# relf/egobox

Hardware: AMD Instinct MI355X
Metric: gp_fixed_theta_fits_per_sec (higher is better)
Workload: dtype f64; 1 GPU; dense GP fixed-theta fit (corr build + Cholesky + likelihood), sq-exp, n=16384 d=32, LHS + Griewank; theta sweep, 192 per step; n=16384, d=32, corr=SquaredExponential, mean=Constant, parallelism=sweep-dp1, fits_in_flight_per_gpu=16, lockstep_width=8

## Files before the change

### egobox_amd/csrc/egx_internal.h

```cpp
#pragma once
#include <hip/hip_runtime.h>
#include <stdint.h>
#include <string>

#include "../../include/egx_gp.h"
#include "schedule.h"

namespace egx {

void set_error(const std::string &msg);
#define EGX_HIP_CHECK(expr)                                                              \
    do {                                                                                 \
        hipError_t _e = (expr);                                                          \
        if (_e != hipSuccess) {                                                          \
            ::egx::set_error(std::string(#expr) + ": " + hipGetErrorString(_e));         \
            (void)hipGetLastError();  \
            return EGX_ERR_HIP;                                                          \
        }                                                                                \
    } while (0)

hipError_t dev_malloc_bytes(void **p, size_t bytes);
template <typename T>
inline hipError_t dev_malloc(T **p, size_t bytes) {
    return dev_malloc_bytes(reinterpret_cast<void **>(p), bytes);
// ... 125 lines not shown
    int rsplit = 1;
    int init = 0;
    const int *active = nullptr;
    double *means = nullptr;
    double *prec = nullptr;
    double *cst = nullptr;
    double *weights = nullptr;
    double *covs = nullptr;
    double *part = nullptr;
    double *lpn_part = nullptr;
    double *lbst = nullptr;
};
inline size_t gmm_part_len(int DP) { return (size_t)(DP / 4) * (DP / 4 + 1) / 2 * kGmmBlockAcc; }
size_t gmm_estep_lds_bytes(int DP, int k);
int launch_gmm_estep(hipStream_t s, const GmmLaunch &g);
int launch_gmm_mstep(hipStream_t s, const GmmLaunch &g, double reg_covar);

inline size_t dinv_doubles(int n_pad) { return (size_t)(n_pad / 64) * 4096 + (size_t)(n_pad / 64); }
struct GemmTrace {
    static constexpr int kMax = 192;
    hipEvent_t e0[kMax], e1[kMax];
    double flops[kMax];
    int used = 0;
    bool ready = false;
};
struct PotrfLookahead {
    hipStream_t s2 = nullptr, s3 = nullptr;
    hipEvent_t ev_lu = nullptr, ev_lur = nullptr, ev_panel = nullptr, ev_a = nullptr, ev_b = nullptr;
};
struct PotrfInverse {
    double *W = nullptr;
    int64_t ldw = 0, sW = 0;
    hipStream_t sw = nullptr;
    hipEvent_t ev_grp = nullptr, ev_done = nullptr;
};
struct GemmBatch {
    int count = 1;
    int64_t sC = 0, sA = 0, sB = 0;
    int sInfo = 0;
};
struct PotrfBatch {
    int count = 1;
    int64_t sM = 0, sD = 0;
    int sI = 0;
    int left = 0;
    int w_left = 0;
    int *sync = nullptr;
    int64_t sS = 0;
    int pipe = 0;
    int whole = 0;
    int flow = 0;
    int flow_tail = 0;
    int group_panels = 0;
    int seqs = 1;
};
int potrf_left_for(int n_pad, int lockstep);
int w_left_for(int n_pad, int lockstep);
PotrfSchedule schedule_for(int n_pad, int lockstep, int n_workspaces);
int potrf_group_panels(int n_pad);
struct TrsmBatch {
    int count = 1;
    int64_t sM = 0, sD = 0, sR = 0;
};
int launch_potrf(hipStream_t s, double *M, int64_t ld, int n_pad, int m_tot, double *dinv, int *info,
                 const PotrfLookahead *lk = nullptr, GemmTrace *trace = nullptr, const PotrfBatch *batch = nullptr,
                 const PotrfInverse *inv = nullptr);
int launch_trsm_rows(hipStream_t s, const double *M, int64_t ldm, int n_pad, const double *dinv,
                     double *RT, int64_t ldr, int m, int tri_rows = 0, const TrsmBatch *batch = nullptr);
int launch_identity_rows(hipStream_t s, double *W, int64_t ld, int n_pad, int count = 1, int64_t stride = 0);
int launch_syrk_uptri_neg(hipStream_t s, double *C, int64_t ldc, const double *W, int64_t ldw, int n,
                          const GemmBatch *batch = nullptr);
int launch_diag_tile_inverses(hipStream_t s, const double *M, int64_t ld, int n_pad, double *dinv);
struct SolveBatchPtrs {
    const double *M[kLockstepMax], *dinv[kLockstepMax];
    double *dW[kLockstepMax], *rhs[kLockstepMax], *vec[kLockstepMax];
};
inline size_t trsv_tail_doubles(int n_pad) { return 4 + (size_t)n_pad; }
inline size_t block_inverse_doubles(int n_pad) { return (size_t)((n_pad + kNB - 1) / kNB) * 65536 + trsv_tail_doubles(n_pad); }
long long pipe_timeout_ticks();
int launch_block_inverse(hipStream_t s, const SolveBatchPtrs &b, int count, int64_t ld, int n_pad);
int launch_trsv_t(hipStream_t s, const SolveBatchPtrs &b, int count, int64_t ld, int n_pad, bool per_block = false);
inline int launch_block_inverse(hipStream_t s, const double *M, int64_t ld, int n_pad, const double *dinv, double *Wall) {
    const SolveBatchPtrs b{{M}, {dinv}, {Wall}, {}, {}};
    return launch_block_inverse(s, b, 1, ld, n_pad);
}
inline int launch_trsv_t(hipStream_t s, const double *M, int64_t ld, int n_pad, double *Wall, double *v, double *xout,
                         bool per_block = false) {
    const SolveBatchPtrs b{{M}, {}, {Wall}, {v}, {xout}};
    return launch_trsv_t(s, b, 1, ld, n_pad, per_block);
}
int launch_gemm_nt_sub(hipStream_t s, double *C, int64_t ldc, const double *A, int64_t lda,
                       const double *B, int64_t ldb, int M, int N, int K, int lower, int ktri = 0,
                       bool *used_big_tile = nullptr, const int *info = nullptr, const GemmBatch *batch = nullptr,
                       int tag = 0);
size_t gram_scratch_doubles(int rows, int K);
int launch_gram_lower(hipStream_t s, const double *W, int64_t ldw, int rows, int K, double *Gneg, int64_t ldg, double *P);
int mfma_probe(double *max_abs_err);

size_t pipe_sync_ints(int n_pad, int m_tot);
int launch_potrf_pipe(hipStream_t s, double *M, int64_t ld, int n_pad, int m_tot, double *dinv, int *info,
                      const PotrfBatch &pb, int g0, int gw, int ext_need = 0, int shared_chip = 0);
int pipe_signal(hipStream_t s, const PotrfBatch &pb, int value);
int launch_potrf_flow(hipStream_t s, double *M, int64_t ld, int n_pad, int m_tot, double *dinv, int *info, const PotrfBatch &pb,
                      int col_base = 0);
bool flow_fits(int n_pad);
int pipe_enabled();
// ... 15 lines not shown
```

### egobox_amd/csrc/gp_host.hip

```cpp
#include "gp_handle.h"
#include "resource_pool.h"

namespace egx {

static thread_local std::string g_last_error;
static std::atomic<int> g_pipe_retry{[] { const char *e = std::getenv("EGX_PIPE_RETRY"); return e ? std::atoi(e) : 1; }()};
static std::atomic<int64_t> g_chain_aborts{0}, g_chain_retries{0};
void set_error(const std::string &msg) { g_last_error = msg; }
const std::string &last_error_string() { return g_last_error; }

}

using namespace egx;

namespace egx {

int set_device(const egx_gp *gp) {
    EGX_HIP_CHECK(hipSetDevice(gp->device));
    return EGX_SUCCESS;
}

struct StreamSet {
    hipStream_t stream = nullptr, inv_stream = nullptr, s2 = nullptr, s3 = nullptr;
};
// ... 278 lines not shown
    }
    egx_gp *gp = owners[0];
    Workspace &lead = *wss[0];
    hipStream_t st = lead.stream;
    PotrfInverse inv;
    if (W0) {
        inv.W = W0;
        inv.ldw = gp->n_pad;
        inv.sW = (int64_t)gp->n_pad * gp->n_pad;
        inv.sw = lead.inv_stream;
        inv.ev_grp = lead.ev_inv_grp;
        inv.ev_done = lead.ev_inv_done;
        EGX_RC(launch_identity_rows(inv.sw, W0, gp->n_pad, gp->n_pad, count, inv.sW));
    }
    for (int j = 0; j < count; j++) {
        Workspace &w = *wss[j];
        w.eval_stream = st;
        std::memcpy(w.h_coef, coefs[j].data(), sizeof(double) * coefs[j].size());
        EGX_HIP_CHECK(hipMemcpyAsync(w.d_coef, w.h_coef, sizeof(double) * coefs[j].size(), hipMemcpyHostToDevice, st));
    }
    EGX_HIP_CHECK(hipMemsetAsync(lead.d_info, 0, sizeof(int) * (size_t)count, st));
    EGX_HIP_CHECK(hipEventRecord(lead.ev[0], st));
    EvalBatchPtrs bp;
    for (int j = 0; j < count; j++) {
        Workspace &w = *wss[j];
        bp.xT[j] = owners[j]->d_xT, bp.coef[j] = w.d_coef, bp.rhsT[j] = owners[j]->d_rhsT, bp.xs[j] = w.d_xs, bp.M[j] = w.M;
        bp.h_diag[j] = w.h_diag, bp.h_rows[j] = w.h_rows, bp.h_info[j] = w.h_info, bp.d_info[j] = w.d_info;
    }
    const int front = launch_eval_front_batch(st, gp->corr, bp, count, gp->n_pad, gp->n, gp->d, hcols, gp->nugget, gp->ld, gp->n_pad,
                                              gp->rhs_pad, gp->q);
    if (front != EGX_SUCCESS && front != EGX_ERR_UNSUPPORTED) return front;
    if (front == EGX_ERR_UNSUPPORTED)
        for (int j = 0; j < count; j++) {
            Workspace &w = *wss[j];
            egx_gp *o = owners[j];
            EGX_RC(launch_corr_sym(st, gp->corr, o->d_xT, gp->n_pad, gp->n, gp->d, w.d_coef, hcols, gp->nugget, w.M, gp->ld,
                                   gp->n_pad, w.d_xs));
            EGX_RC(launch_fill_rows(st, w.M, gp->ld, gp->n_pad, gp->rhs_pad, o->d_rhsT, gp->n_pad, gp->q, gp->n_pad));
        }
    EGX_HIP_CHECK(hipEventRecord(lead.ev[1], st));
    int *lead_sync = dev_sync(gp, (int)(&lead - gp->ws.data()));
    PotrfBatch pb;
    pb.count = count;
    pb.sM = gp->stride_M;
    pb.sD = gp->stride_D;
    pb.sI = 1;
    pb.left = gp->sched.left;
    pb.w_left = gp->sched.w_left;
    pb.pipe = separate ? 0 : gp->sched.pipe;
    pb.whole = separate ? 0 : gp->sched.whole;
    pb.flow = separate || count > 1 || gp->group ? 0 : gp->sched.flow;
    pb.flow_tail = separate || count > 1 || gp->group ? 0 : gp->sched.flow_tail;
    pb.group_panels = gp->sched.group_panels;
    pb.seqs = gp->lockstep > 0 ? ((int)gp->ws.size() + gp->lockstep - 1) / gp->lockstep : 1;
    pb.sync = pb.pipe || pb.flow || pb.flow_tail ? lead_sync : nullptr;
    pb.sS = gp->stride_S;
    for (int j = 0; j < count; j++) {
        wss[j]->retry_hcols = hcols;
        wss[j]->retry_W = W0 ? W0 + (size_t)j * (size_t)gp->n_pad * gp->n_pad : nullptr;
        wss[j]->retry_ncoef = (int)coefs[j].size();
        wss[j]->retried = separate;
    }
    EGX_RC(launch_potrf(st, lead.M, gp->ld, gp->n_pad, gp->m_tot, lead.dinv, lead.d_info, lead.lk.s2 ? &lead.lk : nullptr,
                        &lead.trace, &pb, W0 ? &inv : nullptr));
    EGX_HIP_CHECK(hipEventRecord(lead.ev[2], st));
    EGX_RC(launch_eval_tail(st, bp, count, gp->ld, gp->n, gp->n_pad, gp->q, gp->gls_device ? 0 : 1, pb.sync));
    for (int j = 0; j < count; j++) {
        Workspace &w = *wss[j];
        w.gls_enqueued = gp->gls_device;
        if (gp->gls_device) {
            const int g = gp->rhs_pad;
            EGX_RC(launch_gram_lower(st, w.M + (size_t)gp->n_pad * gp->ld, gp->ld, g, gp->n_pad, w.d_gneg, g, w.d_gramP));
            EGX_RC(launch_gram_finish(st, w.d_gneg, w.d_gram, g, g, gp->q));
            EGX_HIP_CHECK(hipMemsetAsync(w.d_ginfo, 0, sizeof(int), st));
            EGX_RC(launch_potrf(st, w.d_gram, g, g, g, w.d_gdinv, w.d_ginfo));
            EGX_HIP_CHECK(hipMemcpyAsync(w.h_gram, w.d_gram, sizeof(double) * (size_t)g * g, hipMemcpyDeviceToHost, st));
            EGX_HIP_CHECK(hipMemcpyAsync(w.h_ginfo, w.d_ginfo, sizeof(int), hipMemcpyDeviceToHost, st));
        }
        w.sync_lead = pb.sync;
    }
    EGX_HIP_CHECK(hipEventRecord(lead.ev[3], st));
    return EGX_SUCCESS;
}

int enqueue_eval_group(egx_gp *gp, int w0, int count, const std::vector<double> *coefs, int hcols, double *W0) {
    std::vector<egx_gp *> owners((size_t)count, gp);
    std::vector<Workspace *> wss((size_t)count);
    for (int j = 0; j < count; j++) wss[(size_t)j] = &gp->ws[(size_t)(w0 + j)];
    return enqueue_eval_core(owners.data(), wss.data(), count, coefs, hcols, W0);
}
int enqueue_eval_members(egx_gp *const *gps, int count, const std::vector<double> *coefs, int hcols) {
    std::vector<Workspace *> wss((size_t)count);
    for (int j = 0; j < count; j++) wss[(size_t)j] = &gps[j]->ws[0];
    return enqueue_eval_core(gps, wss.data(), count, coefs, hcols, nullptr);
}

int enqueue_eval(egx_gp *gp, Workspace &w, const std::vector<double> &coef, int hcols) {
    return enqueue_eval_group(gp, (int)(&w - gp->ws.data()), 1, &coef, hcols);
}

static int finish_eval_device_gls(egx_gp *gp, Workspace &w, EvalResult &out, int keep) {
    const int n = gp->n, p = gp->p, n_pad = gp->n_pad, g = gp->rhs_pad;
    if (*w.h_ginfo != 0) return 1;
    const double *L = w.h_gram;
    double dmin = std::numeric_limits<double>::infinity(), dmax = 0.0;
    for (int i = 0; i < p; i++) {
// ... 1335 lines not shown
```

### egobox_amd/csrc/kernels_chol.hip

```cpp
#include "egx_internal.h"
#include "dev_mem.h"
#include "potf2_blocks.h"
#include "mfma_gemm_core.h"

#include <atomic>
#include <cstdlib>
#include <mutex>
#include <string>
#include <utility>
#include <vector>

namespace egx {


__device__ __forceinline__ double readlane_d(double v, int lane) {
    union {
        double d;
        int i[2];
    } u;
    u.d = v;
    u.i[0] = __builtin_amdgcn_readlane(u.i[0], lane);
    u.i[1] = __builtin_amdgcn_readlane(u.i[1], lane);
    return u.d;
}
// ... 323 lines not shown
            mma_quarter(a1, b1, 1);
            stage = st1;
        }
#ifdef EGX_STREAM_TRACE
        if (trp) trp[6] = wall_clock64(), trp[7] = clock64();
#endif
#pragma unroll
        for (int r = 0; r < 4; r++) asm volatile("" : "+v"(coff[r]));
#pragma unroll
        for (int mi = 0; mi < 4; mi++)
#pragma unroll
            for (int ni = 0; ni < 4; ni++)
#pragma unroll
                for (int r = 0; r < 4; r++) Ct[(int64_t)mi * 16 * ldc + ni * 16 + coff[r]] = -acc[mi][ni][r];
#ifdef EGX_STREAM_TRACE
        if (trp) {
            asm volatile("s_waitcnt vmcnt(0)" ::: "memory");
            trp[8] = wall_clock64();
        }
#endif
    }
}

#ifdef EGX_STREAM_TRACE
}
extern "C" long long egx_dev_stream_trace(int mode, long long *out, long long cap) {
    static auto &owned = *new egx::DevMem<long long>;
    static long long dcap = 0;
    long long *null = nullptr, *dbuf = owned.p;
    if (mode == 1) {
        owned.reset();
        dcap = cap;
        if (owned.alloc((size_t)(16 + egx::kStraceWords * cap)) != EGX_SUCCESS) return -1;
        dbuf = owned.p;
        (void)hipMemset(dbuf, 0, sizeof(long long) * (16 + egx::kStraceWords * cap));
        (void)hipMemcpy(dbuf + 1, &cap, sizeof(long long), hipMemcpyHostToDevice);
        if (hipMemcpyToSymbol(HIP_SYMBOL(egx::g_strace), &dbuf, sizeof(dbuf)) != hipSuccess) return -2;
        return 0;
    }
    (void)hipDeviceSynchronize();
    (void)hipMemcpyToSymbol(HIP_SYMBOL(egx::g_strace), &null, sizeof(null));
    if (!dbuf) return 0;
    long long taken = 0;
    (void)hipMemcpy(&taken, dbuf, sizeof(long long), hipMemcpyDeviceToHost);
    if (taken > dcap) taken = dcap;
    if (taken > cap) taken = cap;
    if (out && taken > 0) (void)hipMemcpy(out, dbuf + 16, sizeof(long long) * egx::kStraceWords * taken, hipMemcpyDeviceToHost);
    owned.reset();
    return taken;
}
namespace egx {
#endif

constexpr int TS = 64;
constexpr int TLD = 65;

template <int NW>
__device__ __forceinline__ void wg_inv_64(const double *T, const double *rd, double *X, int tid) {
    const int wave = tid >> 6, lane = tid & 63;
    const int frow = lane & 15, fk = lane >> 4;
#pragma unroll 1
    for (int cbk = 3; cbk >= 0; cbk--) {
        for (int rt = wave; rt < 4; rt += NW) {
            double *xt = X + (rt * 16 + fk) * TLD + cbk * 16 + frow;
            double4_t acc = double4_t{0.0, 0.0, 0.0, 0.0};
            if (rt == cbk) {
#pragma unroll
                for (int r = 0; r < 4; r++) acc[r] = (fk + 4 * r == frow) ? 1.0 : 0.0;
            } else if (rt > cbk) {
                for (int kb = cbk + 1; kb <= rt; kb++) {
                    const double *arow = X + (rt * 16 + frow) * TLD + kb * 16 + fk;
                    const double *bcol = T + (kb * 16 + fk) * TLD + cbk * 16 + frow;
#pragma unroll
                    for (int kk = 0; kk < 4; kk++)
                        acc = __builtin_amdgcn_mfma_f64_16x16x4f64(-arow[kk * 4], bcol[(kk * 4) * TLD], acc, 0, 0, 0);
                }
            }
#pragma unroll
            for (int r = 0; r < 4; r++) xt[(4 * r) * TLD] = acc[r];
        }
        __syncthreads();
        if (wave == 0) {
            double x[16];
#pragma unroll
            for (int c = 0; c < 16; c++) x[c] = X[lane * TLD + cbk * 16 + c];
#pragma unroll
            for (int c = 15; c >= 0; c--) {
                double sacc = x[c];
#pragma unroll
                for (int k = c + 1; k < 16; k++)
                    sacc = __builtin_fma(-x[k], T[(cbk * 16 + k) * TLD + cbk * 16 + c], sacc);
                x[c] = sacc * rd[cbk * 16 + c];
            }
#pragma unroll
            for (int c = 0; c < 16; c++) X[lane * TLD + cbk * 16 + c] = x[c];
        }
        __syncthreads();
    }
}


template <int NW>
__global__ __launch_bounds__(64 * NW, 1) void k_potf2_reg(double *__restrict__ D, int64_t ld, int nbk, double *__restrict__ lin,
                                                          int *__restrict__ info, int col0, int n_valid, int64_t bsD,
                                                          int64_t bsL, int bsI) {
    extern __shared__ __attribute__((aligned(16))) double sm[];
// ... 359 lines not shown
                                                        int K, double *__restrict__ P) {
    using S = GemmShape<64, 64, 32, 32, 256>;
    extern __shared__ __attribute__((aligned(16))) double smem[];
    const int t = blockIdx.x;
    int bx = (int)((sqrt(8.0 * t + 1.0) - 1.0) * 0.5);
    while (bx * (bx + 1) / 2 > t) bx--;
    while ((bx + 1) * (bx + 2) / 2 <= t) bx++;
    const int by = t - bx * (bx + 1) / 2;
    const int k0 = blockIdx.y * kc;
    int klen = K - k0;
    if (klen > kc) klen = kc;
    const int tid = threadIdx.x;
    double4_t acc[S::MT][S::NT];
#pragma unroll
    for (int mi = 0; mi < S::MT; mi++)
#pragma unroll
        for (int ni = 0; ni < S::NT; ni++) acc[mi][ni] = double4_t{0.0, 0.0, 0.0, 0.0};
    if (klen > 0)
        gemm_core<64, 64, 32, 32, 256>(W + (int64_t)bx * 64 * ldw + k0, ldw, W + (int64_t)by * 64 * ldw + k0, ldw, klen,
                                       acc, smem, tid);
    const int wave = tid >> 6, lane = tid & 63;
    const int r0 = bx * 64 + (wave / S::WAVES_N) * 32 + (lane >> 4);
    const int c0 = by * 64 + (wave % S::WAVES_N) * 32 + (lane & 15);
    double *out = P + (int64_t)blockIdx.y * rows * rows;
#pragma unroll
    for (int mi = 0; mi < S::MT; mi++)
#pragma unroll
        for (int ni = 0; ni < S::NT; ni++)
#pragma unroll
            for (int r = 0; r < 4; r++) out[(int64_t)(r0 + mi * 16 + 4 * r) * rows + (c0 + ni * 16)] = acc[mi][ni][r];
}

__global__ void k_gram_reduce(const double *__restrict__ P, int rows, int nsplit, double *__restrict__ Gneg, int64_t ldg) {
    const int j = blockIdx.x * blockDim.x + threadIdx.x, i = blockIdx.y;
    if (j >= rows || (j >> 6) > (i >> 6)) return;
    double sacc = 0.0;
    for (int sp = 0; sp < nsplit; sp++) sacc += P[((int64_t)sp * rows + i) * rows + j];
    Gneg[(int64_t)i * ldg + j] = -sacc;
}

static std::atomic<int> g_potrf_group{0};
static std::atomic<int> g_stream_min_tiles{128};
static std::atomic<int> g_gemm_small_max{1024};
static std::atomic<int> g_look_min_cols{3072};
static std::atomic<int> g_lur_side{1};
#ifdef EGX_TEST_HOOKS
static std::atomic<int> g_trsv_stall{0};
#define EGX_TRSV_STALL g_trsv_stall.load()
#else
#define EGX_TRSV_STALL 0
#endif
static std::atomic<int> g_trsv_fused{1};
static std::atomic<int> g_potrf_left{1};
constexpr int kTrsmGroupPanels = 4;
constexpr int kLurSideMinCols = 6144;

int chol_init() {
    static std::once_flag once;
    static int rc_once = EGX_SUCCESS;
    std::call_once(once, [] {
        if (const char *e = std::getenv("EGX_POTRF_GROUP")) {
            const int g = std::atoi(e);
            if (g >= 1 && g <= 8) g_potrf_group = g;
        }
        if (const char *e = std::getenv("EGX_GEMM_SMALL")) g_gemm_small_max = std::atoi(e);
        if (const char *e = std::getenv("EGX_STREAM_MIN")) g_stream_min_tiles = std::atoi(e) > 0 ? std::atoi(e) : 1;
        if (const char *e = std::getenv("EGX_LOOK_MIN")) g_look_min_cols = std::atoi(e);
        if (const char *e = std::getenv("EGX_LUR_SIDE")) g_lur_side = std::atoi(e);
        if (const char *e = std::getenv("EGX_TRSV_FUSED")) g_trsv_fused = std::atoi(e);
        if (const char *e = std::getenv("EGX_POTRF_LEFT")) g_potrf_left = std::atoi(e);
        auto set = [](const void *fn, int bytes) {
            hipError_t e = hipFuncSetAttribute(fn, hipFuncAttributeMaxDynamicSharedMemorySize, bytes);
            if (e != hipSuccess && rc_once == EGX_SUCCESS) {
                set_error(std::string("hipFuncSetAttribute: ") + hipGetErrorString(e));
                rc_once = EGX_ERR_HIP;
            }
        };
        set(reinterpret_cast<const void *>(&k_gemm_nt_sub<true, 128, 128, 32, 64, 512, true>), TrailShape::LDS_BYTES);
        set(reinterpret_cast<const void *>(&k_gemm_nt_sub<false, 128, 128, 32, 64, 512, true>), TrailShape::LDS_BYTES);
        set(reinterpret_cast<const void *>(&k_gemm_stream<true>), ST_LDS_BYTES);
        set(reinterpret_cast<const void *>(&k_gemm_stream<false>), ST_LDS_BYTES);
        set(reinterpret_cast<const void *>(&k_gemm_stream<true, true>), ST_LDS_BYTES);
        set(reinterpret_cast<const void *>(&k_gemm_stream<false, true>), ST_LDS_BYTES);
        set(reinterpret_cast<const void *>(&k_gemm_stream<true, false, 1>), ST_LDS_BYTES);
        set(reinterpret_cast<const void *>(&k_gemm_stream<true, false, 2>), ST_LDS_BYTES);
    });
    return rc_once;
}

static ScheduleKnobs schedule_knobs() {
    (void)chol_init();
    ScheduleKnobs k;
    k.potrf_left = g_potrf_left;
    k.pipe = pipe_enabled();
    k.potrf_group = g_potrf_group;
    return k;
}
int potrf_group_panels(int n_pad) { return schedule_table(n_pad, 1, 1, schedule_knobs()).group_panels; }
PotrfSchedule schedule_for(int n_pad, int lockstep, int n_workspaces) {
    return schedule_table(n_pad, lockstep, n_workspaces, schedule_knobs());
}
int potrf_left_for(int n_pad, int lockstep) { return schedule_for(n_pad, lockstep, 1).left; }
int w_left_for(int n_pad, int lockstep) { return schedule_for(n_pad, lockstep, 1).w_left; }

int set_knob(const char *name, int value) {
    (void)chol_init();
    struct { const char *n; std::atomic<int> *v; } tab[] = {{"potrf_group", &g_potrf_group}, {"stream_min", &g_stream_min_tiles},
                                                           {"gemm_small", &g_gemm_small_max}, {"look_min", &g_look_min_cols},
                                                           {"lur_side", &g_lur_side},         {"potrf_left", &g_potrf_left},
                                                           {"trsv_fused", &g_trsv_fused}};
    for (auto &e : tab)
        if (std::string(name) == e.n) return e.v->exchange(value);
#ifdef EGX_TEST_HOOKS
    if (std::string(name) == "trsv_stall") return g_trsv_stall.exchange(value);
#endif
    return -2147483647 - 1;
}

int launch_gemm_nt_sub(hipStream_t s, double *C, int64_t ldc, const double *A, int64_t lda,
                       const double *B, int64_t ldb, int M, int N, int K, int lower, int ktri, bool *used_big_tile,
                       const int *info, const GemmBatch *batch, int tag) {
    if (used_big_tile) *used_big_tile = false;
    if (M <= 0 || N <= 0 || K <= 0) return EGX_SUCCESS;
    if (M % 128 || N % 128 || K % KC) {
        set_error("gemm_nt_sub: M,N must be multiples of 128 and K of 16");
        return EGX_ERR_INVALID_VALUE;
    }
    const GemmBatch bt = batch ? *batch : GemmBatch();
    const unsigned nz = (unsigned)(bt.count > 0 ? bt.count : 1);
    const int64_t big_tiles = lower ? ((int64_t)(M / 128) * (N / 128) - (int64_t)(N / 128) * (N / 128 - 1) / 2)
                                    : (int64_t)(M / 128) * (N / 128);
    const bool small = big_tiles < g_gemm_small_max;
    int64_t wide_tiles = 0;
    if (N % 256 == 0 && !ktri && (!lower || M >= N)) {
        if (lower)
            for (int c = 0; c < N / 256; c++) wide_tiles += (M / 128 - 2 * c > 0) ? M / 128 - 2 * c : 0;
        else
            wide_tiles = (int64_t)(M / 128) * (N / 256);
    }
    const int64_t min_tiles = (K >= 2048) ? 8 : g_stream_min_tiles.load();
    if (K >= 2 * KC && wide_tiles >= min_tiles) {
        if (used_big_tile) *used_big_tile = wide_tiles >= 512;
        const int nbx = M / 128, nby = N / 256;
        const int nt = (int)wide_tiles;
        const dim3 grid((unsigned)nt, 1, nz);
        if (lower && tag == 1)
            hipLaunchKernelGGL((k_gemm_stream<true, false, 1>), grid, dim3(512), ST_LDS_BYTES, s, C, ldc, A, lda, B, ldb, K, nbx,
                               nby, nt, info, bt);
        else if (lower && tag == 2)
            hipLaunchKernelGGL((k_gemm_stream<true, false, 2>), grid, dim3(512), ST_LDS_BYTES, s, C, ldc, A, lda, B, ldb, K, nbx,
                               nby, nt, info, bt);
        else if (lower)
            hipLaunchKernelGGL((k_gemm_stream<true>), grid, dim3(512), ST_LDS_BYTES, s, C, ldc, A, lda, B, ldb, K, nbx, nby, nt,
                               info, bt);
        else
            hipLaunchKernelGGL((k_gemm_stream<false>), grid, dim3(512), ST_LDS_BYTES, s, C, ldc, A, lda, B, ldb, K, nbx, nby, nt,
                               info, bt);
        EGX_HIP_CHECK(hipGetLastError());
        return EGX_SUCCESS;
    }
    if (small) {
        const dim3 grid(M / 64, N / 64, nz);
        if (lower)
            hipLaunchKernelGGL((k_gemm_nt_sub<true, 64, 64, 32, 32, 256, false>), grid, dim3(256), SmallShape::LDS_BYTES, s,
                               C, ldc, A, lda, B, ldb, K, M / 64, N / 64, ktri, info, bt);
        else
            hipLaunchKernelGGL((k_gemm_nt_sub<false, 64, 64, 32, 32, 256, false>), grid, dim3(256), SmallShape::LDS_BYTES,
                               s, C, ldc, A, lda, B, ldb, K, M / 64, N / 64, ktri, info, bt);
    } else {
        const int nbx = M / 128, nby = N / 128;
        const int nsx = (nbx + 7) / 8, nsy = (nby + 7) / 8;
        int nst;
        if (lower) {
            const int tri_rows = nsx < nsy ? nsx : nsy;
            nst = tri_rows * (tri_rows + 1) / 2 + (nsx > nsy ? (nsx - nsy) * nsy : 0);
            if (nsx < nsy) nst = nsy * (nsy + 1) / 2;
        } else {
            nst = nsx * nsy;
        }
        const int per_xcd = (nst + 7) / 8;
        const dim3 grid(8 * per_xcd * 64, 1, nz);
        if (lower)
            hipLaunchKernelGGL((k_gemm_nt_sub<true, 128, 128, 32, 64, 512, true>), grid, dim3(512), TrailShape::LDS_BYTES, s,
                               C, ldc, A, lda, B, ldb, K, nbx, nby, ktri, info, bt);
        else
            hipLaunchKernelGGL((k_gemm_nt_sub<false, 128, 128, 32, 64, 512, true>), grid, dim3(512), TrailShape::LDS_BYTES,
                               s, C, ldc, A, lda, B, ldb, K, nbx, nby, ktri, info, bt);
    }
    EGX_HIP_CHECK(hipGetLastError());
    return EGX_SUCCESS;
}

static int gram_nsplit(int rows, int K) {
    const int nt = rows / 64, tiles = nt * (nt + 1) / 2;
    int nsplit = (2048 + tiles - 1) / tiles;
    const int maxs = K / 512 > 0 ? K / 512 : 1;
    if (nsplit > maxs) nsplit = maxs;
    if (nsplit < 1) nsplit = 1;
    return nsplit;
}
size_t gram_scratch_doubles(int rows, int K) { return (size_t)gram_nsplit(rows, K) * rows * rows; }
int launch_gram_lower(hipStream_t s, const double *W, int64_t ldw, int rows, int K, double *Gneg, int64_t ldg, double *P) {
    if (rows % 64 || K % KC) {
        set_error("gram: rows must be a multiple of 64 and K of 16");
        return EGX_ERR_INVALID_VALUE;
    }
    const int nt = rows / 64, tiles = nt * (nt + 1) / 2;
    int nsplit = gram_nsplit(rows, K);
    int kc = (int)round_up((K + nsplit - 1) / nsplit, 128);
    nsplit = (K + kc - 1) / kc;
    hipLaunchKernelGGL(k_gram_splitk, dim3(tiles, nsplit), dim3(256), SmallShape::LDS_BYTES, s, W, ldw, rows, kc, K, P);
    hipLaunchKernelGGL(k_gram_reduce, dim3((rows + 255) / 256, rows), dim3(256), 0, s, (const double *)P, rows, nsplit, Gneg,
                       ldg);
    EGX_HIP_CHECK(hipGetLastError());
    return EGX_SUCCESS;
}

int launch_potrf(hipStream_t s, double *M, int64_t ld, int n_pad, int m_tot, double *dinv, int *info,
                 const PotrfLookahead *lk, GemmTrace *trace, const PotrfBatch *batch, const PotrfInverse *inv) {
    if (trace) trace->used = 0;
    int rc = chol_init();
    if (rc) return rc;
    if (n_pad % kTile || m_tot % kTile || m_tot < n_pad) {
        set_error("potrf: padded sizes must be multiples of 128");
        return EGX_ERR_INVALID_VALUE;
    }
    const PotrfBatch pb = batch ? *batch : PotrfBatch();
    const unsigned nz = (unsigned)(pb.count > 0 ? pb.count : 1);
    GemmBatch gb;
    gb.count = (int)nz;
    gb.sC = gb.sA = gb.sB = pb.sM;
    gb.sInfo = pb.sI;
    hipStream_t s2 = lk ? lk->s2 : nullptr, s3 = lk ? lk->s3 : nullptr;
    auto potf2 = [&](hipStream_t st, int k0, int nbk) {
        double *diag = M + (int64_t)k0 * ld + k0;
        double *dtiles = dinv + (int64_t)(k0 / 64) * 4096;
        hipLaunchKernelGGL(k_potf2_reg<16>, dim3(1, 1, nz), dim3(1024), RB_LDS_BYTES, st, diag, ld, nbk, dtiles, info, k0, n_pad,
                           pb.sM, pb.sD, pb.sI);
    };
    auto trsm = [&](hipStream_t st, int k0, int nbk) {
        const int below = m_tot - (k0 + nbk);
        if (below <= 0) return;
        double *P = M + (int64_t)(k0 + nbk) * ld + k0;
        const double *L = M + (int64_t)k0 * ld + k0;
        const double *lin = dinv + (int64_t)(k0 / 64) * 4096;
        if (below >= 4096)
            hipLaunchKernelGGL((k_panel_trsm16<2, false>), dim3(below / 32, 1, nz), dim3(256), 0, st, P, ld, L, ld, lin, nbk,
                               (const int *)info, pb.sM, pb.sM, pb.sD, pb.sI, (const double *)nullptr);
        else
            hipLaunchKernelGGL((k_panel_trsm16<1, false>), dim3(below / 16, 1, nz), dim3(256), 0, st, P, ld, L, ld, lin, nbk,
                               (const int *)info, pb.sM, pb.sM, pb.sD, pb.sI, (const double *)nullptr);
    };
    auto update = [&](hipStream_t st, int r0, int c0, int Mr, int N, int k0, int K, int lower, bool *big, int tag = 0) -> int {
        return launch_gemm_nt_sub(st, M + (int64_t)r0 * ld + c0, ld, M + (int64_t)r0 * ld + k0, ld,
                                  M + (int64_t)c0 * ld + k0, ld, Mr, N, K, lower, 0, big, info, &gb, tag);
    };
    const int GW = (pb.group_panels > 0 ? pb.group_panels : potrf_group_panels(n_pad)) * kNB;
    const bool flow = pb.sync != nullptr && pb.flow != 0 && nz == 1 && inv == nullptr && flow_fits(n_pad);
    const int tail_cols = (pb.sync != nullptr && pb.flow_tail > 0 && nz == 1 && inv == nullptr && !pb.left && pb.flow_tail < n_pad && (n_pad - pb.flow_tail) % GW == 0 &&
                           flow_fits(pb.flow_tail))
                              ? pb.flow_tail
                              : 0;
    const bool have_sync = flow || tail_cols > 0 || (pb.sync != nullptr && pb.pipe != 0 &&
                                    pipe_fits((int)nz, ((pb.whole || GW > n_pad ? n_pad : GW) + kNB - 1) / kNB));
    const bool pipe = have_sync && !flow && tail_cols == 0;
    if (have_sync) EGX_HIP_CHECK(hipMemsetAsync(pb.sync, 0, sizeof(int) * (nz > 1 ? (size_t)pb.sS * nz : pipe_sync_ints(n_pad, m_tot)), s));
    auto gwidth = [&](int g0) { return (n_pad - g0 < GW) ? (n_pad - g0) : GW; };
    auto inner_factor = [&](hipStream_t st, int g0, int gw, hipStream_t side, hipEvent_t first_wait) -> int {
        if (pipe) {
            const bool on_device = first_wait != nullptr && pb.seqs <= 2;
            if (first_wait && !on_device) EGX_HIP_CHECK(hipStreamWaitEvent(st, first_wait, 0));
            const int rc2 = launch_potrf_pipe(st, M, ld, n_pad, m_tot, dinv, info, pb, g0, gw, on_device ? g0 / kNB + 1 : 0, st != s);
            if (rc2 == EGX_SUCCESS && on_device) EGX_HIP_CHECK(hipStreamWaitEvent(st, first_wait, 0));
            return rc2;
        }
        hipEvent_t pending = first_wait;
        for (int k0 = g0; k0 < g0 + gw; k0 += kNB) {
            const int nbk = (g0 + gw - k0 < kNB) ? (g0 + gw - k0) : kNB;
            potf2(st, k0, nbk);
            if (pending) {
                EGX_HIP_CHECK(hipStreamWaitEvent(st, pending, 0));
                pending = nullptr;
            }
            trsm(st, k0, nbk);
            const int r1 = k0 + nbk;
            if (r1 >= g0 + gw) break;
            const int ncols = g0 + gw - r1;
            const int nb1 = ncols < kNB ? ncols : kNB;
            const int rest_rows = m_tot - r1 - nb1;
            if (side && rest_rows >= 128) {
                int rc2 = update(st, r1, r1, nb1, nb1, k0, nbk, 1, nullptr);
                if (rc2) return rc2;
                EGX_HIP_CHECK(hipEventRecord(lk->ev_a, st));
                EGX_HIP_CHECK(hipStreamWaitEvent(side, lk->ev_a, 0));
                rc2 = update(side, r1 + nb1, r1, rest_rows, ncols, k0, nbk, 0, nullptr);
                if (rc2) return rc2;
                EGX_HIP_CHECK(hipEventRecord(lk->ev_b, side));
                pending = lk->ev_b;
            } else {
                int rc2 = update(st, r1, r1, m_tot - r1, ncols, k0, nbk, 1, nullptr);
                if (rc2) return rc2;
            }
        }
        if (pending) EGX_HIP_CHECK(hipStreamWaitEvent(st, pending, 0));
        return EGX_SUCCESS;
    };
    GemmBatch gbw;
    if (inv) {
// ... 22 lines not shown
                hipLaunchKernelGGL((k_panel_trsm16<1, false>), dim3(m_eff / 16, 1, nz), dim3(256), 0, sw, P, inv->ldw, L, ld, lin, nbk,
                                   (const int *)info, inv->sW, pb.sM, pb.sD, pb.sI, (const double *)nullptr);
            const int ncols = gend - (k0 + nbk);
            if (ncols > 0) {
                int rc2 = launch_gemm_nt_sub(sw, inv->W + (k0 + nbk), inv->ldw, inv->W + k0, inv->ldw,
                                             M + (int64_t)(k0 + nbk) * ld + k0, ld, m_eff, ncols, nbk, 0, 0, nullptr, info, &gbw);
                if (rc2) return rc2;
            }
        }
        const int ncols = n_pad - gend;
        if (ncols > 0 && w_left) {
            const int gwn = gwidth(gend);
            const int nbx = gend / 128, nby = gwn / 256, nt = nbx * nby;
            hipLaunchKernelGGL((k_gemm_stream<false, true>), dim3((unsigned)nt * nz, 1, 1), dim3(512), ST_LDS_BYTES, sw, inv->W + gend,
                               inv->ldw, (const double *)inv->W, inv->ldw, (const double *)(M + (int64_t)gend * ld), ld, gend, nbx,
                               nby, nt, (const int *)info, gbw);
            EGX_HIP_CHECK(hipGetLastError());
        } else if (ncols > 0) {
            int rc2 = launch_gemm_nt_sub(sw, inv->W + gend, inv->ldw, inv->W + g0, inv->ldw, M + (int64_t)gend * ld + g0, ld, gend,
                                         ncols, gw, 0, 0, nullptr, info, &gbw);
            if (rc2) return rc2;
        }
        return EGX_SUCCESS;
    };
    if (flow || (pipe && pb.whole)) {
        rc = flow ? launch_potrf_flow(s, M, ld, n_pad, m_tot, dinv, info, pb) : launch_potrf_pipe(s, M, ld, n_pad, m_tot, dinv, info, pb, 0, n_pad);
        if (rc) return rc;
        if (inv) {
            for (int g0 = 0; g0 < n_pad; g0 += GW) {
                rc = inverse_group(s, g0, gwidth(g0));
                if (rc) return rc;
            }
            EGX_HIP_CHECK(hipEventRecord(inv->ev_done, inv->sw));
            EGX_HIP_CHECK(hipStreamWaitEvent(s, inv->ev_done, 0));
        }
        hipLaunchKernelGGL(k_diag_tile_inverses, dim3(n_pad / 64, 1, nz), dim3(256), 0, s, (const double *)M, ld, dinv,
                           dinv + (int64_t)(n_pad / 64) * 4096, pb.sM, pb.sD);
        EGX_HIP_CHECK(hipGetLastError());
        return EGX_SUCCESS;
    }
    if (pb.left) {
        const bool la = s2 != nullptr;
        hipStream_t sc = la ? s2 : s;
        rc = inner_factor(s, 0, gwidth(0), s3, nullptr);
        if (rc) return rc;
        rc = inverse_group(s, 0, gwidth(0));
        if (rc) return rc;
        int gprev = 0;
        for (int g0 = gwidth(0); g0 < n_pad; g0 += GW) {
            const int gw = gwidth(g0);
            if (gprev > 0) {
                const bool timed = trace && trace->ready && trace->used < GemmTrace::kMax;
                if (timed) EGX_HIP_CHECK(hipEventRecord(trace->e0[trace->used], s));
                rc = update(s, g0, g0, m_tot - g0, gw, 0, gprev, 1, nullptr, 1);
                if (rc) return rc;
                if (timed) {
                    EGX_HIP_CHECK(hipEventRecord(trace->e1[trace->used], s));
                    const double nr = (double)(n_pad - g0);
                    trace->flops[trace->used] = (double)nz * 2.0 * gprev * (nr * gw - 0.5 * gw * (gw - 1.0));
                    trace->used++;
                }
            }
            if (la && gprev > 0) EGX_HIP_CHECK(hipStreamWaitEvent(s, lk->ev_panel, 0));
            rc = update(s, g0, g0, m_tot - g0, gw, gprev, g0 - gprev, 1, nullptr, 2);
            if (rc) return rc;
            if (la) {
                EGX_HIP_CHECK(hipEventRecord(lk->ev_lu, s));
                EGX_HIP_CHECK(hipStreamWaitEvent(sc, lk->ev_lu, 0));
            }
            rc = inner_factor(sc, g0, gw, la ? s3 : nullptr, nullptr);
            if (rc) return rc;
            if (la) EGX_HIP_CHECK(hipEventRecord(lk->ev_panel, sc));
            rc = inverse_group(sc, g0, gw);
            if (rc) return rc;
            gprev = g0;
        }
        if (la && gprev > 0) EGX_HIP_CHECK(hipStreamWaitEvent(s, lk->ev_panel, 0));
        if (inv) {
            EGX_HIP_CHECK(hipEventRecord(inv->ev_done, inv->sw));
            EGX_HIP_CHECK(hipStreamWaitEvent(s, inv->ev_done, 0));
        }
        hipLaunchKernelGGL(k_diag_tile_inverses, dim3(n_pad / 64, 1, nz), dim3(256), 0, s, (const double *)M, ld, dinv,
                           dinv + (int64_t)(n_pad / 64) * 4096, pb.sM, pb.sD);
        EGX_HIP_CHECK(hipGetLastError());
        return EGX_SUCCESS;
    }
    rc = inner_factor(s, 0, gwidth(0), s3, nullptr);
    if (rc) return rc;
    rc = inverse_group(s, 0, gwidth(0));
    if (rc) return rc;
    for (int g0 = 0; g0 < n_pad; g0 += GW) {
        const int gw = gwidth(g0);
        const int r1 = g0 + gw;
        if (r1 >= n_pad) break;
        const int gw1 = gwidth(r1);
        if (tail_cols > 0 && n_pad - r1 == tail_cols) {
            rc = update(s, r1, r1, m_tot - r1, n_pad - r1, g0, gw, 1, nullptr);
            if (rc) return rc;
            rc = launch_potrf_flow(s, M + (int64_t)r1 * ld + r1, ld, n_pad - r1, m_tot - r1, dinv + (int64_t)(r1 / 64) * 4096, info, pb, r1);
            if (rc) return rc;
            for (int t0 = r1; t0 < n_pad; t0 += GW) {
                rc = inverse_group(s, t0, gwidth(t0));
                if (rc) return rc;
            }
            break;
        }
        const bool look = (s2 != nullptr) && (n_pad - r1 - gw1 >= g_look_min_cols);
        const int nb1 = gw1 < kNB ? gw1 : kNB;
        if (look && s3) {
            rc = update(s, r1, r1, nb1, nb1, g0, gw, 1, nullptr);
            if (rc) return rc;
            EGX_HIP_CHECK(hipEventRecord(lk->ev_lu, s));
            EGX_HIP_CHECK(hipStreamWaitEvent(s2, lk->ev_lu, 0));
            hipStream_t slu = (g_lur_side && n_pad >= 14336 && n_pad - r1 - gw1 >= kLurSideMinCols) ? s3 : s;
            if (slu != s) EGX_HIP_CHECK(hipStreamWaitEvent(slu, lk->ev_lu, 0));
            rc = update(slu, r1 + nb1, r1, m_tot - r1 - nb1, gw1, g0, gw, 0, nullptr);
            if (rc) return rc;
            EGX_HIP_CHECK(hipEventRecord(lk->ev_lur, slu));
            if (pipe) {
                rc = pipe_signal(slu, pb, r1 / kNB + 1);
                if (rc) return rc;
            }
            rc = inner_factor(s2, r1, gw1, s3, lk->ev_lur);
            if (rc) return rc;
            EGX_HIP_CHECK(hipEventRecord(lk->ev_panel, s2));
        } else if (!look) {
            const bool timed = trace && trace->ready && trace->used < GemmTrace::kMax;
            if (timed) EGX_HIP_CHECK(hipEventRecord(trace->e0[trace->used], s));
            bool big = false;
            rc = update(s, r1, r1, m_tot - r1, n_pad - r1, g0, gw, 1, &big);
            if (rc) return rc;
            if (timed && big) {
                EGX_HIP_CHECK(hipEventRecord(trace->e1[trace->used], s));
                const double nc = (double)(n_pad - r1);
                trace->flops[trace->used] = (double)nz * 2.0 * gw * nc * (nc + 1.0) / 2.0;
                trace->used++;
            }
        } else {
            rc = update(s, r1, r1, m_tot - r1, gw1, g0, gw, 1, nullptr);
            if (rc) return rc;
            EGX_HIP_CHECK(hipEventRecord(lk->ev_lu, s));
            EGX_HIP_CHECK(hipStreamWaitEvent(s2, lk->ev_lu, 0));
            rc = inner_factor(s2, r1, gw1, nullptr, nullptr);
            if (rc) return rc;
            EGX_HIP_CHECK(hipEventRecord(lk->ev_panel, s2));
        }
        const int r2 = r1 + gw1;
        if (r2 < n_pad && look) {
            const bool timed = trace && trace->ready && trace->used < GemmTrace::kMax;
            if (timed) EGX_HIP_CHECK(hipEventRecord(trace->e0[trace->used], s));
            bool big = false;
            rc = update(s, r2, r2, m_tot - r2, n_pad - r2, g0, gw, 1, &big);
            if (rc) return rc;
            if (timed && big) {
                EGX_HIP_CHECK(hipEventRecord(trace->e1[trace->used], s));
                const double nc = (double)(n_pad - r2);
                trace->flops[trace->used] = (double)nz * 2.0 * gw * nc * (nc + 1.0) / 2.0;
                trace->used++;
            }
        }
        if (look) {
            EGX_HIP_CHECK(hipStreamWaitEvent(s, lk->ev_panel, 0));
        } else {
            rc = inner_factor(s, r1, gw1, nullptr, nullptr);
            if (rc) return rc;
        }
        rc = inverse_group(s, r1, gw1);
        if (rc) return rc;
    }
    if (inv) {
        EGX_HIP_CHECK(hipEventRecord(inv->ev_done, inv->sw));
        EGX_HIP_CHECK(hipStreamWaitEvent(s, inv->ev_done, 0));
    }
    hipLaunchKernelGGL(k_diag_tile_inverses, dim3(n_pad / 64, 1, nz), dim3(256), 0, s, (const double *)M, ld, dinv,
                       dinv + (int64_t)(n_pad / 64) * 4096, pb.sM, pb.sD);
    EGX_HIP_CHECK(hipGetLastError());
    return EGX_SUCCESS;
}

int launch_trsm_rows(hipStream_t s, const double *M, int64_t ldm, int n_pad, const double *dinv, double *RT,
                     int64_t ldr, int m, int tri_rows, const TrsmBatch *batch) {
    int rc = chol_init();
    if (rc) return rc;
    const TrsmBatch tb = batch ? *batch : TrsmBatch();
    const unsigned nz = (unsigned)(tb.count > 0 ? tb.count : 1);
    GemmBatch gb;
    gb.count = (int)nz;
    gb.sC = gb.sA = tb.sR;
    gb.sB = tb.sM;
    if (m % kTile || n_pad % kTile) {
        set_error("trsm_rows: sizes must be multiples of 128");
        return EGX_ERR_INVALID_VALUE;
    }
    const int GW = kTrsmGroupPanels * kNB;
    const bool left = !tri_rows;
    for (int g0 = 0; g0 < n_pad; g0 += GW) {
        const int gw = (n_pad - g0 < GW) ? (n_pad - g0) : GW;
        const int gend = g0 + gw;
        if (left && g0 > 0) {
            rc = launch_gemm_nt_sub(s, RT + g0, ldr, RT, ldr, M + (int64_t)g0 * ldm, ldm, m, gw, g0, 0, 0, nullptr, nullptr, &gb);
            if (rc) return rc;
        }
        for (int k0 = g0; k0 < gend; k0 += kNB) {
            const int nbk = (gend - k0 < kNB) ? (gend - k0) : kNB;
            const double *diag = M + (int64_t)k0 * ldm + k0;
            const double *dtiles = dinv + (int64_t)(k0 / 64) * 4096;
            const int m_eff = tri_rows ? ((k0 + nbk < m) ? (k0 + nbk) : m) : m;
            const double *tfl = dinv + (int64_t)(n_pad / 64) * 4096 + k0 / 64;
// ... 141 lines not shown
```

Before: 42.62 fits/s.

## Update RHS rows in Cholesky trailing GEMM with a thin 16-row strip kernel

The trailing update in the blocked Cholesky also covers the appended RHS rows, which are padded to a full 128-row block. The streaming GEMM now stops at n_pad rows, and a new MFMA f64 strip kernel handles only the real RHS rows (q ≤ 64) in 16-row tiles with register prefetch. This avoids wasted FLOPs on padding rows at the cost of one extra kernel launch per update. Trace event recording moves into the update lambda so timing still brackets the big GEMM only.

```diff
diff --git a/egobox_amd/csrc/egx_internal.h b/egobox_amd/csrc/egx_internal.h
--- a/egobox_amd/csrc/egx_internal.h
+++ b/egobox_amd/csrc/egx_internal.h
@@ -201,6 +201,7 @@
     int flow = 0;
     int flow_tail = 0;
     int group_panels = 0;
+    int rhs_rows = 0;
     int seqs = 1;
 };
 int potrf_left_for(int n_pad, int lockstep);
diff --git a/egobox_amd/csrc/gp_host.hip b/egobox_amd/csrc/gp_host.hip
--- a/egobox_amd/csrc/gp_host.hip
+++ b/egobox_amd/csrc/gp_host.hip
@@ -354,6 +354,7 @@
     pb.flow = separate || count > 1 || gp->group ? 0 : gp->sched.flow;
     pb.flow_tail = separate || count > 1 || gp->group ? 0 : gp->sched.flow_tail;
     pb.group_panels = gp->sched.group_panels;
+    pb.rhs_rows = gp->q;
     pb.seqs = gp->lockstep > 0 ? ((int)gp->ws.size() + gp->lockstep - 1) / gp->lockstep : 1;
     pb.sync = pb.pipe || pb.flow || pb.flow_tail ? lead_sync : nullptr;
     pb.sS = gp->stride_S;
diff --git a/egobox_amd/csrc/kernels_chol.hip b/egobox_amd/csrc/kernels_chol.hip
--- a/egobox_amd/csrc/kernels_chol.hip
+++ b/egobox_amd/csrc/kernels_chol.hip
@@ -399,6 +399,64 @@
 namespace egx {
 #endif
 
+constexpr int kStripAhead = 8;
+__global__ __launch_bounds__(256) void k_gemm_strip16(double *C, int64_t ldc, const double *A, int64_t lda, const double *B, int64_t ldb,
+                                                      int K, const int *__restrict__ info, GemmBatch bt) {
+    {
+        const int64_t z = blockIdx.z;
+        C += z * bt.sC;
+        A += z * bt.sA;
+        B += z * bt.sB;
+        if (info != nullptr) info += z * bt.sInfo;
+    }
+    if (wg_failed_before(info)) return;
+    const int tid = threadIdx.x, lane = tid & 63, frow = lane & 15, fk = lane >> 4;
+    const int wave = __builtin_amdgcn_readfirstlane(tid >> 6);
+    const int row0 = (int)blockIdx.y * 16, col0 = ((int)blockIdx.x * 4 + wave) * 16;
+    const double *pa = A + (int64_t)(row0 + frow) * lda + 2 * fk;
+    const double *pb = B + (int64_t)(col0 + frow) * ldb + 2 * fk;
+    double *Cw = C + (int64_t)(row0 + fk) * ldc + col0 + frow;
+    double4_t acc;
+#pragma unroll
+    for (int r = 0; r < 4; r++) acc[r] = -Cw[(int64_t)(4 * r) * ldc];
+    const int nch = K / KC;
+    d2_t ra[kStripAhead][2], rb[kStripAhead][2];
+    auto fetch = [&](int slot, int ch) {
+#pragma unroll
+        for (int kb = 0; kb < 2; kb++) {
+            ra[slot][kb] = *reinterpret_cast<const d2_t *>(pa + ch * KC + 8 * kb);
+            rb[slot][kb] = *reinterpret_cast<const d2_t *>(pb + ch * KC + 8 * kb);
+        }
+        asm volatile("" ::: "memory");
+    };
+    auto mma_chunk = [&](const d2_t (&a)[2], const d2_t (&b)[2]) {
+#pragma unroll
+        for (int kb = 0; kb < 2; kb++) {
+            acc = __builtin_amdgcn_mfma_f64_16x16x4f64(a[kb][0], b[kb][0], acc, 0, 0, 0);
+            acc = __builtin_amdgcn_mfma_f64_16x16x4f64(a[kb][1], b[kb][1], acc, 0, 0, 0);
+        }
+    };
+    const int nring = nch - nch % kStripAhead;
+    if (nring > 0) {
+#pragma unroll
+        for (int i = 0; i < kStripAhead; i++) fetch(i, i);
+    }
+    for (int c = 0; c < nring; c += kStripAhead) {
+#pragma unroll
+        for (int i = 0; i < kStripAhead; i++) {
+            mma_chunk(ra[i], rb[i]);
+            const int cn = c + kStripAhead + i;
+            fetch(i, cn < nring ? cn : nring - 1);
+        }
+    }
+    for (int c = nring; c < nch; c++) {
+        fetch(0, c);
+        mma_chunk(ra[0], rb[0]);
+    }
+#pragma unroll
+    for (int r = 0; r < 4; r++) Cw[(int64_t)(4 * r) * ldc] = -acc[r];
+}
+
 constexpr int TS = 64;
 constexpr int TLD = 65;
 
@@ -864,6 +922,7 @@
 #endif
 static std::atomic<int> g_trsv_fused{1};
 static std::atomic<int> g_potrf_left{1};
+static std::atomic<int> g_rhs_strip{1};
 constexpr int kTrsmGroupPanels = 4;
 constexpr int kLurSideMinCols = 6144;
 
@@ -881,6 +940,7 @@
         if (const char *e = std::getenv("EGX_LUR_SIDE")) g_lur_side = std::atoi(e);
         if (const char *e = std::getenv("EGX_TRSV_FUSED")) g_trsv_fused = std::atoi(e);
         if (const char *e = std::getenv("EGX_POTRF_LEFT")) g_potrf_left = std::atoi(e);
+        if (const char *e = std::getenv("EGX_RHS_STRIP")) g_rhs_strip = std::atoi(e);
         auto set = [](const void *fn, int bytes) {
             hipError_t e = hipFuncSetAttribute(fn, hipFuncAttributeMaxDynamicSharedMemorySize, bytes);
             if (e != hipSuccess && rc_once == EGX_SUCCESS) {
@@ -920,7 +980,7 @@
     struct { const char *n; std::atomic<int> *v; } tab[] = {{"potrf_group", &g_potrf_group}, {"stream_min", &g_stream_min_tiles},
                                                            {"gemm_small", &g_gemm_small_max}, {"look_min", &g_look_min_cols},
                                                            {"lur_side", &g_lur_side},         {"potrf_left", &g_potrf_left},
-                                                           {"trsv_fused", &g_trsv_fused}};
+                                                           {"trsv_fused", &g_trsv_fused},     {"rhs_strip", &g_rhs_strip}};
     for (auto &e : tab)
         if (std::string(name) == e.n) return e.v->exchange(value);
 #ifdef EGX_TEST_HOOKS
@@ -929,20 +989,7 @@
     return -2147483647 - 1;
 }
 
-int launch_gemm_nt_sub(hipStream_t s, double *C, int64_t ldc, const double *A, int64_t lda,
-                       const double *B, int64_t ldb, int M, int N, int K, int lower, int ktri, bool *used_big_tile,
-                       const int *info, const GemmBatch *batch, int tag) {
-    if (used_big_tile) *used_big_tile = false;
-    if (M <= 0 || N <= 0 || K <= 0) return EGX_SUCCESS;
-    if (M % 128 || N % 128 || K % KC) {
-        set_error("gemm_nt_sub: M,N must be multiples of 128 and K of 16");
-        return EGX_ERR_INVALID_VALUE;
-    }
-    const GemmBatch bt = batch ? *batch : GemmBatch();
-    const unsigned nz = (unsigned)(bt.count > 0 ? bt.count : 1);
-    const int64_t big_tiles = lower ? ((int64_t)(M / 128) * (N / 128) - (int64_t)(N / 128) * (N / 128 - 1) / 2)
-                                    : (int64_t)(M / 128) * (N / 128);
-    const bool small = big_tiles < g_gemm_small_max;
+static int64_t stream_wide_tiles(int M, int N, int lower, int ktri) {
     int64_t wide_tiles = 0;
     if (N % 256 == 0 && !ktri && (!lower || M >= N)) {
         if (lower)
@@ -950,11 +997,31 @@
         else
             wide_tiles = (int64_t)(M / 128) * (N / 256);
     }
+    return wide_tiles;
+}
+static bool takes_stream(int M, int N, int K, int lower, int ktri) {
     const int64_t min_tiles = (K >= 2048) ? 8 : g_stream_min_tiles.load();
-    if (K >= 2 * KC && wide_tiles >= min_tiles) {
-        if (used_big_tile) *used_big_tile = wide_tiles >= 512;
-        const int nbx = M / 128, nby = N / 256;
-        const int nt = (int)wide_tiles;
+    return M > 0 && N > 0 && M % 128 == 0 && N % 128 == 0 && K % KC == 0 && K >= 2 * KC && stream_wide_tiles(M, N, lower, ktri) >= min_tiles;
+}
+static int gemm_nt_sub_rows(hipStream_t s, double *C, int64_t ldc, const double *A, int64_t lda, const double *B, int64_t ldb, int M,
+                            int N, int K, int lower, int ktri, bool *used_big_tile, const int *info, const GemmBatch *batch, int tag,
+                            int m_stream) {
+    if (used_big_tile) *used_big_tile = false;
+    if (M <= 0 || N <= 0 || K <= 0) return EGX_SUCCESS;
+    if (M % 128 || N % 128 || K % KC) {
+        set_error("gemm_nt_sub: M,N must be multiples of 128 and K of 16");
+        return EGX_ERR_INVALID_VALUE;
+    }
+    const GemmBatch bt = batch ? *batch : GemmBatch();
+    const unsigned nz = (unsigned)(bt.count > 0 ? bt.count : 1);
+    const int64_t big_tiles = lower ? ((int64_t)(M / 128) * (N / 128) - (int64_t)(N / 128) * (N / 128 - 1) / 2)
+                                    : (int64_t)(M / 128) * (N / 128);
+    const bool small = big_tiles < g_gemm_small_max;
+    if (takes_stream(M, N, K, lower, ktri)) {
+        if (used_big_tile) *used_big_tile = stream_wide_tiles(M, N, lower, ktri) >= 512;
+        const int nbx = m_stream / 128, nby = N / 256;
+        const int nt = (int)stream_wide_tiles(m_stream, N, lower, ktri);
+        if (nt <= 0) return EGX_SUCCESS;
         const dim3 grid((unsigned)nt, 1, nz);
         if (lower && tag == 1)
             hipLaunchKernelGGL((k_gemm_stream<true, false, 1>), grid, dim3(512), ST_LDS_BYTES, s, C, ldc, A, lda, B, ldb, K, nbx,
@@ -1001,6 +1068,12 @@
     }
     EGX_HIP_CHECK(hipGetLastError());
     return EGX_SUCCESS;
+}
+
+int launch_gemm_nt_sub(hipStream_t s, double *C, int64_t ldc, const double *A, int64_t lda,
+                       const double *B, int64_t ldb, int M, int N, int K, int lower, int ktri, bool *used_big_tile,
+                       const int *info, const GemmBatch *batch, int tag) {
+    return gemm_nt_sub_rows(s, C, ldc, A, lda, B, ldb, M, N, K, lower, ktri, used_big_tile, info, batch, tag, M);
 }
 
 static int gram_nsplit(int rows, int K) {
@@ -1063,9 +1136,23 @@
             hipLaunchKernelGGL((k_panel_trsm16<1, false>), dim3(below / 16, 1, nz), dim3(256), 0, st, P, ld, L, ld, lin, nbk,
                                (const int *)info, pb.sM, pb.sM, pb.sD, pb.sI, (const double *)nullptr);
     };
-    auto update = [&](hipStream_t st, int r0, int c0, int Mr, int N, int k0, int K, int lower, bool *big, int tag = 0) -> int {
-        return launch_gemm_nt_sub(st, M + (int64_t)r0 * ld + c0, ld, M + (int64_t)r0 * ld + k0, ld,
-                                  M + (int64_t)c0 * ld + k0, ld, Mr, N, K, lower, 0, big, info, &gb, tag);
+    const int rhs_pad = m_tot - n_pad;
+    const bool strips = g_rhs_strip.load() != 0 && rhs_pad > 0 && pb.rhs_rows > 0 && pb.rhs_rows <= 64;
+    auto update = [&](hipStream_t st, int r0, int c0, int Mr, int N, int k0, int K, int lower, bool *big, int tag = 0,
+                      hipEvent_t e1 = nullptr) -> int {
+        double *C = M + (int64_t)r0 * ld + c0;
+        const double *A = M + (int64_t)r0 * ld + k0, *B = M + (int64_t)c0 * ld + k0;
+        const bool strip = strips && r0 <= n_pad && r0 + Mr == m_tot && takes_stream(Mr, N, K, lower, 0);
+        const int rc2 = gemm_nt_sub_rows(st, C, ld, A, ld, B, ld, Mr, N, K, lower, 0, big, info, &gb, tag, strip ? Mr - rhs_pad : Mr);
+        if (rc2) return rc2;
+        if (e1 && (!big || *big)) EGX_HIP_CHECK(hipEventRecord(e1, st));
+        if (strip) {
+            const int64_t rows_above = (int64_t)(n_pad - r0) * ld;
+            hipLaunchKernelGGL(k_gemm_strip16, dim3((unsigned)(N / 64), (unsigned)((pb.rhs_rows + 15) / 16), nz), dim3(256), 0, st,
+                               C + rows_above, ld, A + rows_above, ld, B, ld, K, (const int *)info, gb);
+            EGX_HIP_CHECK(hipGetLastError());
+        }
+        return EGX_SUCCESS;
     };
     const int GW = (pb.group_panels > 0 ? pb.group_panels : potrf_group_panels(n_pad)) * kNB;
     const bool flow = pb.sync != nullptr && pb.flow != 0 && nz == 1 && inv == nullptr && flow_fits(n_pad);
@@ -1194,10 +1281,9 @@
             if (gprev > 0) {
                 const bool timed = trace && trace->ready && trace->used < GemmTrace::kMax;
                 if (timed) EGX_HIP_CHECK(hipEventRecord(trace->e0[trace->used], s));
-                rc = update(s, g0, g0, m_tot - g0, gw, 0, gprev, 1, nullptr, 1);
+                rc = update(s, g0, g0, m_tot - g0, gw, 0, gprev, 1, nullptr, 1, timed ? trace->e1[trace->used] : nullptr);
                 if (rc) return rc;
                 if (timed) {
-                    EGX_HIP_CHECK(hipEventRecord(trace->e1[trace->used], s));
                     const double nr = (double)(n_pad - g0);
                     trace->flops[trace->used] = (double)nz * 2.0 * gprev * (nr * gw - 0.5 * gw * (gw - 1.0));
                     trace->used++;
@@ -1270,10 +1356,9 @@
             const bool timed = trace && trace->ready && trace->used < GemmTrace::kMax;
             if (timed) EGX_HIP_CHECK(hipEventRecord(trace->e0[trace->used], s));
             bool big = false;
-            rc = update(s, r1, r1, m_tot - r1, n_pad - r1, g0, gw, 1, &big);
+            rc = update(s, r1, r1, m_tot - r1, n_pad - r1, g0, gw, 1, &big, 0, timed ? trace->e1[trace->used] : nullptr);
             if (rc) return rc;
             if (timed && big) {
-                EGX_HIP_CHECK(hipEventRecord(trace->e1[trace->used], s));
                 const double nc = (double)(n_pad - r1);
                 trace->flops[trace->used] = (double)nz * 2.0 * gw * nc * (nc + 1.0) / 2.0;
                 trace->used++;
@@ -1292,10 +1377,9 @@
             const bool timed = trace && trace->ready && trace->used < GemmTrace::kMax;
             if (timed) EGX_HIP_CHECK(hipEventRecord(trace->e0[trace->used], s));
             bool big = false;
-            rc = update(s, r2, r2, m_tot - r2, n_pad - r2, g0, gw, 1, &big);
+            rc = update(s, r2, r2, m_tot - r2, n_pad - r2, g0, gw, 1, &big, 0, timed ? trace->e1[trace->used] : nullptr);
             if (rc) return rc;
             if (timed && big) {
-                EGX_HIP_CHECK(hipEventRecord(trace->e1[trace->used], s));
                 const double nc = (double)(n_pad - r2);
                 trace->flops[trace->used] = (double)nz * 2.0 * gw * nc * (nc + 1.0) / 2.0;
                 trace->used++;
```

Result: no change. 42.77 fits/s (median of 6 runs) (+0.3%).
